# sczhou/CodeFormer

Hardware: AMD Instinct MI355X
Metric: aligned 512x512 faces/sec (whole node) at w=0.5 (higher is better)
Workload: dtype f32; 1 GPU; BASELINE config 2 (IEEE fp32 arithmetic): 16 faces/GPU, w=0.5, adain, seed-0 random-init weights; global_batch=16, parallelism=single GPU, precision=fp32

## Files before the change

### codeformer_amd/csrc/cf_wf43.hip

```cpp
#include <cstdlib>
#include <cstring>
#include <type_traits>

#include "cf_conv_parts.h"




namespace {

constexpr int F4_TH = 16, F4_TW = 16;
constexpr int F4_PW = F4_TW + 2;
constexpr int F4_NPIX = (F4_TH + 2) * F4_PW;
constexpr int F4_SLOTS = F4_NPIX + 4;
constexpr int F4_DUMMY = F4_NPIX;
constexpr int F4_NT = 16;
constexpr int F4_PATCH_FLOATS = F4_SLOTS * CF_BK;
constexpr int F4_PS = F4_NT * CF_BK;
constexpr int F4_V_FLOATS = 36 * F4_PS;
constexpr int F4_M_FLOATS = 36 * 8 * 64;
constexpr int F4_TAB = 256;
constexpr int F4_TAB_32 = 512;
constexpr int F4_LDS_FLOATS = 2 * F4_PATCH_FLOATS + F4_V_FLOATS + 2 * F4_TAB;
static_assert(F4_M_FLOATS <= 2 * F4_PATCH_FLOATS + F4_V_FLOATS, "epilogue staging must fit the patch buffers + V");
static_assert(F4_LDS_FLOATS * 4 <= 81920, "LDS budget of two workgroups per CU");
constexpr int F4_LDS_FLOATS_16 = 2 * F4_M_FLOATS;
static_assert(F4_LDS_FLOATS_16 >= F4_LDS_FLOATS && F4_LDS_FLOATS_16 * 4 <= 163840, "LDS budget of the 16-wave form");
constexpr int F4_LDS_FLOATS_32 = 2 * F4_SLOTS * 32 + 36 * F4_NT * 32 + 2 * F4_TAB_32;
static_assert(F4_LDS_FLOATS_32 >= F4_LDS_FLOATS_16 && F4_LDS_FLOATS_32 * 4 <= 163840, "LDS budget of the 32-channel-slab form");

typedef _Float16 f4_f16x4 __attribute__((ext_vector_type(4)));
typedef float f4_f32x2 __attribute__((ext_vector_type(2)));
typedef unsigned f4_u32x4 __attribute__((ext_vector_type(4)));
typedef unsigned f4_u32x2 __attribute__((ext_vector_type(2)));

__device__ __forceinline__ __amdgpu_buffer_rsrc_t f4_rsrc(const void* p, unsigned bytes) {
  return __builtin_amdgcn_make_buffer_rsrc(const_cast<void*>(p), 0, bytes, 0x00020000);
}
__device__ __forceinline__ f32x4 f4_ld128(__amdgpu_buffer_rsrc_t r, unsigned voff, unsigned soff) {
  return __builtin_bit_cast(f32x4, __builtin_amdgcn_raw_buffer_load_b128(r, (int)voff, (int)soff, 0));
}
__device__ __forceinline__ f4_f32x2 f4_ld64(__amdgpu_buffer_rsrc_t r, unsigned voff, unsigned soff) {
  return __builtin_bit_cast(f4_f32x2, __builtin_amdgcn_raw_buffer_load_b64(r, (int)voff, (int)soff, 0));
}
__device__ __forceinline__ void f4_st64(f4_f32x2 v, __amdgpu_buffer_rsrc_t r, unsigned voff, unsigned soff) {
  __builtin_amdgcn_raw_buffer_store_b64(__builtin_bit_cast(f4_u32x2, v), r, (int)voff, (int)soff, 0);
}

struct F4Args {
  const float* in0;
  const float* in1;
  int c0, c1, cin, nchunks;
  int batch, h, w;
  int cout;
  int prologue, epilogue;
  const float* pro_scale;
  const float* pro_shift;
  const float* weight;
  const float* bias;
  const float* res;
  const float* sft_scale;
  float sft_w;
  float acc_scale;
  const float* sft_w_img;
  const float* act_scale;
  float* out;
  double* stats_out;
  int stats_cpg, nparts;
  int tiles_x, tiles_per_img, ntn;
  int nt_out;
};
static_assert(sizeof(F4Args) == 168, "the kernarg block is 168 bytes (160 before sft_w_img, which found no padding to take): its size feeds the register allocation of every instantiation, so a change is re-checked with tools/kernel_resources.py");

__device__ __forceinline__ int f4_vs(int ty) { return (0x78 >> (2 * ty)) & 3; }

__device__ __forceinline__ unsigned f4_vu(unsigned lq, unsigned p, unsigned t) { return (lq & 1u) + 2u * (((t >> 1) + 4u * (lq >> 1) + p) & 7u); }

template <int PRO, int EPI, int NW, int KS, bool F32, int UPF = 0>
__global__ __launch_bounds__(NW * 64, 4) void wf43_kernel(const F4Args a) {
  constexpr bool UP = UPF == 2;
  constexpr bool GUP = UPF == 1;
  static_assert(UPF == 0 || (F32 && NW == 16 && KS == 32 && PRO == CF_PRO_NONE && EPI == CF_EPI_NONE), "the upsampling forms: fp32 operands on 32-channel slabs, no prologue, no epilogue operand");
  constexpr int NPW = UP ? 13 : 18;
  constexpr int NXI = UP ? 5 : 6;
  constexpr int OS = UP ? 2 : 1;
  static_assert(KS == 16 || (KS == 32 && NW == 16), "32-channel slabs need the LDS of the 16-wave form");
  constexpr int F4_THREADS = NW * 64;
  constexpr int F4_BN = NW * 8;
  constexpr int TWV = KS / 4;
  constexpr int QPP = KS / 4;
  constexpr int GT = F4_THREADS - TWV * 64;
  constexpr int F4_APT = 384 * QPP / GT;
  constexpr int PSTEP = GT / QPP;
  constexpr int SLOTB = KS * 4;
  constexpr int PATCHF = F4_SLOTS * KS;
  constexpr int PSK = F4_NT * KS;
  extern __shared__ __attribute__((aligned(16))) float smem[];
  float* const V = smem + 2 * PATCHF;
  constexpr int VBUF = 36 * PSK;
  constexpr int TABN = KS == 32 ? F4_TAB_32 : F4_TAB;
  float* const tab = V + VBUF;

  const int tid = threadIdx.x;
  const int lane = tid & 63;
  const int wave = __builtin_amdgcn_readfirstlane(tid >> 6);

  const int bid = cf_xcd_tile(blockIdx.x, gridDim.x);
  const int ntile = bid % a.ntn;
  const int mt = bid / a.ntn;
  const int n0 = ntile * F4_BN;
  const int b = mt / a.tiles_per_img;
  const int rt = mt - b * a.tiles_per_img;
  const int blocks = a.tiles_per_img >> 2;
  const int phase = UP ? rt / blocks : 0;
  const int pa = phase >> 1, pb = phase & 1;
  const int blk = UP ? rt - phase * blocks : rt;
  const int tyw = blk / a.tiles_x;
  const int y0 = tyw * F4_TH;
  const int x0 = (blk - tyw * a.tiles_x) * F4_TW;
  const int n = a.cin / KS;

  constexpr bool affine = PRO == CF_PRO_AFFINE || PRO == CF_PRO_AFFINE_SWISH;
  if (affine) {
    for (int i = tid; i < a.cin; i += F4_THREADS) {
      tab[i] = a.pro_scale[(size_t)b * a.cin + i];
      tab[TABN + i] = a.pro_shift[(size_t)b * a.cin + i];
    }
  }
  float act_s, act_is, act_s02;
  cf_act_scales<!affine>(a.act_scale, b, act_s, act_is, act_s02);

  const int py0 = y0 - 1 + pa, px0 = x0 - 1 + pb;
  const int pix_origin = py0 * a.w + px0;
  auto item = [&](unsigned u, int j, unsigned& rel, bool& valid) __attribute__((always_inline)) {
    const unsigned p = u + (unsigned)(PSTEP * j);
    const unsigned hy = (p * 3641u) >> 16;
    const unsigned hx = p - 18u * hy;
    const int iy = py0 + (int)hy, ix = px0 + (int)hx;
    valid = (int)(p < (unsigned)F4_NPIX) & (int)((unsigned)iy < (unsigned)a.h) & (int)((unsigned)ix < (unsigned)a.w);
    if constexpr (GUP) {
      const unsigned sy = valid ? (unsigned)iy : (unsigned)(y0 + 8), sx = valid ? (unsigned)ix : (unsigned)(x0 + 8);
      rel = (sy >> 1) * ((unsigned)a.w >> 1) + (sx >> 1);
    } else {
      rel = valid ? hy * (unsigned)a.w + hx : (unsigned)(9 * a.w + 9);
    }
  };
  const size_t img0 = (size_t)b * a.h * a.w;
  const unsigned img_px = (unsigned)(a.h * a.w);
  const size_t img0_in = GUP ? img0 / 4 : img0;
  const unsigned img_px_in = GUP ? img_px / 4 : img_px;
  const __amdgpu_buffer_rsrc_t rs_in0 = f4_rsrc(a.in0 + img0_in * a.c0, img_px_in * (unsigned)a.c0 * 4u);
  const __amdgpu_buffer_rsrc_t rs_in1 = f4_rsrc(a.c1 ? a.in1 + img0_in * a.c1 : a.in0, img_px_in * (unsigned)a.c1 * 4u);
  constexpr bool HALVES = F4_APT >= 6;
  constexpr int RAN = HALVES ? F4_APT / 2 : F4_APT;
  f32x4 ra[RAN], rb[HALVES ? RAN : 1];
  auto load_A_range = [&](int chunk, auto j0c, auto j1c) __attribute__((always_inline)) {
    constexpr int J0 = decltype(j0c)::value, J1 = decltype(j1c)::value;
    const int c = chunk * KS;
    const bool first = c < a.c0;
    const unsigned cs = (unsigned)(first ? a.c0 : a.c1);
    const unsigned soff = (unsigned)(first ? c : c - a.c0) * 4u;
    unsigned tl = (unsigned)tid - (unsigned)(TWV * 64);
    asm volatile("" : "+v"(tl));
    const unsigned k4x = (tl % (unsigned)QPP) * 4u;
#pragma unroll
    for (int j = J0; j < J1; ++j) {
      unsigned rel;
      bool valid;
      item(tl / (unsigned)QPP, j, rel, valid);
      const unsigned voff = (__umul24(GUP ? rel : (unsigned)(pix_origin + (int)rel), cs) + k4x) * 4u;
      (HALVES && j >= RAN ? rb[j % RAN] : ra[j % RAN]) = first ? f4_ld128(rs_in0, voff, soff) : f4_ld128(rs_in1, voff, soff);
    }
  };
  auto load_A = [&](int chunk) __attribute__((always_inline)) { load_A_range(chunk, std::integral_constant<int, 0>{}, std::integral_constant<int, F4_APT>{}); };
  auto store_patch_range = [&](int chunk, auto j0c, auto j1c) __attribute__((always_inline)) {
    constexpr int J0 = decltype(j0c)::value, J1 = decltype(j1c)::value;
    unsigned tl = (unsigned)tid - (unsigned)(TWV * 64);
    asm volatile("" : "+v"(tl));
    const unsigned k4 = tl % (unsigned)QPP, slot = tl / (unsigned)QPP;
    char* const pb = reinterpret_cast<char*>(smem + (chunk & 1) * PATCHF) + (((slot & ~3u) | ((slot ^ (slot >> 2)) & 3u)) * (unsigned)SLOTB + k4 * 16u);
    f32x4 sc = {1.f, 1.f, 1.f, 1.f}, sh = {0.f, 0.f, 0.f, 0.f};
    if (affine) {
      sc = *reinterpret_cast<const f32x4*>(tab + chunk * KS + k4 * 4);
      sh = *reinterpret_cast<const f32x4*>(tab + TABN + chunk * KS + k4 * 4);
    }
#pragma unroll
    for (int j = J0; j < J1; ++j) {
      unsigned rel;
      bool valid;
      item(slot, j, rel, valid);
      const f32x4 v = cf_pro_apply4<PRO, true>(HALVES && j >= RAN ? rb[j % RAN] : ra[j % RAN], sc, sh, act_s, act_s02, valid);
      if (j < F4_APT - 1 || slot + (unsigned)(PSTEP * j) < (unsigned)F4_NPIX) *reinterpret_cast<f32x4*>(pb + j * (PSTEP * SLOTB)) = v;
    }
  };

  auto store_patch = [&](int chunk) __attribute__((always_inline)) { store_patch_range(chunk, std::integral_constant<int, 0>{}, std::integral_constant<int, F4_APT>{}); };

  const int tg = (wave >> (KS == 32 ? 2 : 1)) & 1;
  float* t_hi;
  float* t_lo;
  auto row_pass = [&](const f4_f32x2 (&zz)[6], int pos) __attribute__((always_inline)) {
    f4_f32x2 v[6];
    v[0] = (zz[0] + zz[4]) * 0.25f - zz[2] * 1.0625f;
    const f4_f32x2 e1 = zz[4] * 0.25f - zz[2];
    const f4_f32x2 o1 = zz[3] * 0.125f - zz[1] * 0.5f;
    v[1] = e1 + o1;
    v[2] = e1 - o1;
    const f4_f32x2 e2 = zz[4] * 0.5f - zz[2] * 0.125f;
    const f4_f32x2 o2 = zz[3] - zz[1] * 0.25f;
    v[3] = e2 + o2;
    v[4] = e2 - o2;
    v[5] = (zz[1] + zz[5]) * 0.25f - zz[3] * 1.0625f;
#pragma unroll
    for (int nu = 0; nu < 6; ++nu) {
      if (F32) {
        t_hi[(pos + nu) * PSK] = v[nu][0];
        t_lo[(pos + nu) * PSK] = v[nu][1];
      } else {
        float hi, lo;
        cf_split_pair(v[nu][0], v[nu][1], hi, lo);
        t_hi[(pos + nu) * PSK] = hi;
        t_lo[(pos + nu) * PSK] = lo;
      }
    }
  };
  auto bt42 = [](auto xi, f4_f32x2 d0, f4_f32x2 d1, f4_f32x2 d2, f4_f32x2 d3, f4_f32x2 d4) __attribute__((always_inline)) {
    constexpr int XI = decltype(xi)::value;
    if constexpr (XI == 0) return (d0 + d3) - (d1 + d2) * 1.5f;
    else if constexpr (XI == 1) return (d1 + d3) - d2 * 2.5f;
    else if constexpr (XI == 2) return (d3 - d2) - d1 * 2.f;
    else if constexpr (XI == 3) return (d2 - d1) * 0.5f + d3;
    else return (d1 + d4) - (d2 + d3) * 1.5f;
  };
  auto row_pass42 = [&](const f4_f32x2 (&zz)[5], int pos) __attribute__((always_inline)) {
    f4_f32x2 v[5];
    v[0] = bt42(std::integral_constant<int, 0>{}, zz[0], zz[1], zz[2], zz[3], zz[4]);
    v[1] = bt42(std::integral_constant<int, 1>{}, zz[0], zz[1], zz[2], zz[3], zz[4]);
    v[2] = bt42(std::integral_constant<int, 2>{}, zz[0], zz[1], zz[2], zz[3], zz[4]);
    v[3] = bt42(std::integral_constant<int, 3>{}, zz[0], zz[1], zz[2], zz[3], zz[4]);
    v[4] = bt42(std::integral_constant<int, 4>{}, zz[0], zz[1], zz[2], zz[3], zz[4]);
#pragma unroll
    for (int nu = 0; nu < 5; ++nu) {
      t_hi[(pos + nu) * PSK] = v[nu][0];
      t_lo[(pos + nu) * PSK] = v[nu][1];
    }
  };
  auto transform = [&](int chunk, auto mid) __attribute__((always_inline)) {
    const char* const pb = reinterpret_cast<const char*>(smem + (chunk & 1) * PATCHF);
    unsigned ln = (unsigned)lane;
    asm volatile("" : "+v"(ln));
    constexpr int TG0 = UP ? 15 : 18;
    const unsigned t_tile = KS == 32 ? 4u * (unsigned)(wave & 3) + (ln >> 4) : 8u * (unsigned)(wave & 1) + (ln >> 3);
    const unsigned t_cp = KS == 32 ? ln & 15u : ln & 7u;
    const unsigned t_ty = t_tile >> 2, t_tx = t_tile & 3u;
    constexpr unsigned SH = KS == 32 ? 7 : 6;
    const unsigned t_base = (4u << SH) * (18u * t_ty + t_tx) + t_cp * 8u;
    const unsigned tb0 = 2u * t_ty + t_tx;
    unsigned tk[4];
#pragma unroll
    for (int k = 0; k < 4; ++k) tk[k] = t_base | (((tb0 + k) & 3u) << SH);
    if (F32) {
      const unsigned lq0 = (2u * t_cp) & 3u, j = t_cp >> 1;
      if (KS == 32) {
        t_hi = V + (tg * TG0) * PSK + t_tile * 32 + f4_vu(lq0, j >> 1, t_tile) * 2u + (j & 1u);
        t_lo = V + (tg * TG0) * PSK + t_tile * 32 + f4_vu(lq0 + 1u, j >> 1, t_tile) * 2u + (j & 1u);
      } else {
        t_hi = V + (tg * TG0) * PSK + t_tile * CF_BK + ((lq0 ^ (unsigned)f4_vs((int)t_ty)) << 2) + j;
        t_lo = V + (tg * TG0) * PSK + t_tile * CF_BK + (((lq0 + 1u) ^ (unsigned)f4_vs((int)t_ty)) << 2) + j;
      }
    } else if (KS == 32) {
      const unsigned lq = t_cp >> 2, e = t_cp & 3u;
      t_hi = V + (tg * TG0) * PSK + t_tile * 32 + f4_vu(lq, e >> 1, t_tile) * 2u + (e & 1u);
      t_lo = V + (tg * TG0) * PSK + t_tile * 32 + f4_vu(lq, 2u + (e >> 1), t_tile) * 2u + (e & 1u);
    } else {
      t_hi = V + (tg * TG0) * PSK + t_tile * CF_BK + (((t_cp >> 1) ^ (unsigned)f4_vs((int)t_ty)) << 2) + (t_cp & 1u);
      t_lo = t_hi + 2;
    }
    auto px = [&](int r, int j) __attribute__((always_inline)) {
      const int q = 2 * r + j;
      return *reinterpret_cast<const f4_f32x2*>(pb + (4 << SH) * (4 * r + (q >> 2)) + (tk[q >> 2] ^ (((unsigned)q & 3u) << SH)));
    };
    if constexpr (UP) {
      auto xi_pass = [&](auto xi) __attribute__((always_inline)) {
        constexpr int XI = decltype(xi)::value;
        f4_f32x2 z[5];
#pragma unroll
        for (int j = 0; j < 5; ++j) {
          const f4_f32x2 zero = {0.f, 0.f};
          z[j] = bt42(xi, XI == 0 ? px(0, j) : zero, px(1, j), px(2, j), px(3, j), XI == 4 ? px(4, j) : zero);
        }
        __builtin_amdgcn_sched_barrier(0);
        row_pass42(z, (XI >= 3 ? XI - 3 : XI) * 5);
        __builtin_amdgcn_sched_barrier(0);
      };
      if (tg == 0) {
        xi_pass(std::integral_constant<int, 0>{});
        xi_pass(std::integral_constant<int, 1>{});
        mid();
        __builtin_amdgcn_sched_barrier(0);
        xi_pass(std::integral_constant<int, 2>{});
      } else {
        xi_pass(std::integral_constant<int, 3>{});
        mid();
        __builtin_amdgcn_sched_barrier(0);
        xi_pass(std::integral_constant<int, 4>{});
      }
    } else if (tg == 0) {
      {
        f4_f32x2 z[6];
#pragma unroll
        for (int j = 0; j < 6; ++j) z[j] = (px(0, j) + px(4, j)) * 0.25f - px(2, j) * 1.0625f;
        __builtin_amdgcn_sched_barrier(0);
        row_pass(z, 0);
      }
      __builtin_amdgcn_sched_barrier(0);
      {
        f4_f32x2 zp[6], zm[6];
#pragma unroll
        for (int j = 0; j < 6; ++j) {
          const f4_f32x2 e = px(4, j) * 0.25f - px(2, j);
          const f4_f32x2 o = px(3, j) * 0.125f - px(1, j) * 0.5f;
          zp[j] = e + o;
          zm[j] = e - o;
          if (j == 2) __builtin_amdgcn_sched_barrier(0);
        }
        __builtin_amdgcn_sched_barrier(0);
        row_pass(zp, 6);
        __builtin_amdgcn_sched_barrier(0);
        mid();
        __builtin_amdgcn_sched_barrier(0);
        row_pass(zm, 12);
      }
    } else {
      {
        f4_f32x2 z[6];
#pragma unroll
        for (int j = 0; j < 6; ++j) z[j] = (px(1, j) + px(5, j)) * 0.25f - px(3, j) * 1.0625f;
        __builtin_amdgcn_sched_barrier(0);
        row_pass(z, 12);
      }
      __builtin_amdgcn_sched_barrier(0);
      {
        f4_f32x2 zp[6], zm[6];
#pragma unroll
        for (int j = 0; j < 6; ++j) {
          const f4_f32x2 e = px(4, j) * 0.5f - px(2, j) * 0.125f;
          const f4_f32x2 o = px(3, j) - px(1, j) * 0.25f;
          zp[j] = e + o;
          zm[j] = e - o;
          if (j == 2) __builtin_amdgcn_sched_barrier(0);
        }
        __builtin_amdgcn_sched_barrier(0);
        row_pass(zp, 0);
        __builtin_amdgcn_sched_barrier(0);
        mid();
        __builtin_amdgcn_sched_barrier(0);
        row_pass(zm, 6);
      }
    }
  };

  const int m_g = wave / (NW / 2), m_nb = wave % (NW / 2);
  f32x4 acc[NPW];
#pragma unroll
  for (int i = 0; i < NPW; ++i) acc[i] = f32x4{0.f, 0.f, 0.f, 0.f};
  const __amdgpu_buffer_rsrc_t rs_w = f4_rsrc(a.weight, (UP ? 100u : 36u) * (unsigned)a.cin * (unsigned)a.cout * 4u);
  const unsigned w_pos = (unsigned)a.cin * (unsigned)a.cout * 4u;
  const unsigned w_chunk = (unsigned)(a.cout * KS) * 4u;
  const unsigned w_s0 = (unsigned)(18 * m_g) * w_pos + (unsigned)(n0 / 16 + m_nb) * (unsigned)(64 * KS);
  constexpr std::integral_constant<int, 4> nb4{};
  unsigned lane16;
  f32x4 bq[4];
  auto load_B = [&](int chunk, int i, auto nb) __attribute__((always_inline)) {
    bq[i % decltype(nb)::value] = f4_ld128(rs_w, lane16, w_s0 + (unsigned)i * w_pos + (unsigned)chunk * w_chunk);
  };
  auto set_lane16 = [&]() __attribute__((always_inline)) {
    unsigned ln = (unsigned)lane;
    asm volatile("" : "+v"(ln));
    lane16 = ln * 16u;
  };
  const float* a_base;
  f32x4 va[4];
  auto mfma = [&](float a0, float a1, float b0, float b1, f32x4& c) __attribute__((always_inline)) {
    c = __builtin_amdgcn_mfma_f32_16x16x16f16(__builtin_bit_cast(f4_f16x4, f4_f32x2{a0, a1}), __builtin_bit_cast(f4_f16x4, f4_f32x2{b0, b1}), c, 0, 0, 0);
  };
  auto mma_stage = [&](int chunk, auto na, auto after_last_B) __attribute__((always_inline)) {
    constexpr int NA = decltype(na)::value;
    {
      unsigned ln = (unsigned)lane;
      asm volatile("" : "+v"(ln));
      const unsigned t15 = ln & 15u;
      a_base = V + (18 * m_g) * PSK + t15 * CF_BK + (((ln >> 4) ^ (unsigned)f4_vs((int)(t15 >> 2))) << 2);
      lane16 = ln * 16u;
    }
    auto read_A = [&](int i) __attribute__((always_inline)) { va[i % NA] = *reinterpret_cast<const f32x4*>(a_base + i * PSK); };
    read_A(0);
    read_A(1);
#pragma unroll
    for (int i = 0; i < 18; i += 2) {
      if (NA == 4 && i + 2 < 18) {
        read_A(i + 2);
        read_A(i + 3);
      }
      __builtin_amdgcn_sched_barrier(0);
      const f32x4 a0 = va[i % NA], a1 = va[(i + 1) % NA], b0 = bq[i % 4], b1 = bq[(i + 1) % 4];
      if (F32) {
#pragma unroll
        for (int j = 0; j < 4; ++j) {
          acc[i] = __builtin_amdgcn_mfma_f32_16x16x4f32(a0[j], b0[j], acc[i], 0, 0, 0);
          acc[i + 1] = __builtin_amdgcn_mfma_f32_16x16x4f32(a1[j], b1[j], acc[i + 1], 0, 0, 0);
        }
      } else {
        mfma(a0[2], a0[3], b0[0], b0[1], acc[i]);
        mfma(a1[2], a1[3], b1[0], b1[1], acc[i + 1]);
        mfma(a0[0], a0[1], b0[2], b0[3], acc[i]);
        mfma(a1[0], a1[1], b1[2], b1[3], acc[i + 1]);
        mfma(a0[0], a0[1], b0[0], b0[1], acc[i]);
        mfma(a1[0], a1[1], b1[0], b1[1], acc[i + 1]);
      }
      if (NA == 2 && i + 2 < 18) {
        read_A(i + 2);
        read_A(i + 3);
      }
      if (i + 4 < 18) {
        load_B(chunk, i + 4, nb4);
        load_B(chunk, i + 5, nb4);
      }
      if (i + 4 == 16) after_last_B();
      __builtin_amdgcn_sched_barrier(0);
    }
  };
  typedef _Float16 f4_f16x8 __attribute__((ext_vector_type(8)));
  f32x4 xb[3][2], xa[1][2];
  const int p_g = NPW * m_g;
  const int p_nb = m_nb;
  const bool p_last = !UP || m_g == 0;
  const unsigned w_s32 = (unsigned)(p_g + 25 * phase) * w_pos + (unsigned)(n0 / 16 + p_nb) * (unsigned)(64 * KS);
  auto load_B32 = [&](int chunk, int i) __attribute__((always_inline)) {
    const unsigned so = w_s32 + (unsigned)i * w_pos + (unsigned)chunk * w_chunk;
    xb[i % 3][0] = f4_ld128(rs_w, lane16, so);
    xb[i % 3][1] = f4_ld128(rs_w, lane16 + 16u, so);
  };
  auto mma_stage32 = [&](int chunk) __attribute__((always_inline)) {
    unsigned ao[4];
    {
      unsigned ln = (unsigned)lane;
      asm volatile("" : "+v"(ln));
      const unsigned t15 = ln & 15u, lq = ln >> 4;
#pragma unroll
      for (unsigned pp = 0; pp < 4; ++pp) ao[pp] = ((unsigned)p_g * (unsigned)PSK + t15 * 32u + f4_vu(lq, pp, t15) * 2u) * 4u;
      lane16 = ln * 32u;
    }
    const char* const vb = reinterpret_cast<const char*>(V);
    auto read_A = [&](int pos) __attribute__((always_inline)) {
      const f4_f32x2 p0 = *reinterpret_cast<const f4_f32x2*>(vb + ao[0] + pos * (PSK * 4)), p1 = *reinterpret_cast<const f4_f32x2*>(vb + ao[1] + pos * (PSK * 4));
      const f4_f32x2 p2 = *reinterpret_cast<const f4_f32x2*>(vb + ao[2] + pos * (PSK * 4)), p3 = *reinterpret_cast<const f4_f32x2*>(vb + ao[3] + pos * (PSK * 4));
      xa[0][0] = f32x4{p0[0], p0[1], p1[0], p1[1]};
      xa[0][1] = f32x4{p2[0], p2[1], p3[0], p3[1]};
    };
    auto mf = [&](f32x4 av, f32x4 bv, f32x4& c) __attribute__((always_inline)) {
      c = __builtin_amdgcn_mfma_f32_16x16x32_f16(__builtin_bit_cast(f4_f16x8, av), __builtin_bit_cast(f4_f16x8, bv), c, 0, 0, 0);
    };
    read_A(0);
#pragma unroll
    for (int i = 0; i < NPW; ++i) {
      __builtin_amdgcn_sched_barrier(0);
      if (F32) {
        if (i + 1 < NPW || p_last) {
#pragma unroll
          for (int j = 0; j < 8; ++j) {
            acc[i] = __builtin_amdgcn_mfma_f32_16x16x4f32(xa[0][j >> 2][j & 3], xb[i % 3][j >> 2][j & 3], acc[i], 0, 0, 0);
          }
        }
      } else {
        mf(xa[0][1], xb[i % 3][0], acc[i]);
        mf(xa[0][0], xb[i % 3][1], acc[i]);
        mf(xa[0][0], xb[i % 3][0], acc[i]);
      }
      if (i + 1 < NPW && (p_last || i + 1 < NPW - 1)) read_A(i + 1);
      if (i + 3 < NPW && (p_last || i + 3 < NPW - 1)) load_B32(chunk, i + 3);
      __builtin_amdgcn_sched_barrier(0);
    }
  };
  auto set_lane32 = [&]() __attribute__((always_inline)) {
    unsigned ln = (unsigned)lane;
    asm volatile("" : "+v"(ln));
    lane16 = ln * 32u;
  };
  constexpr std::integral_constant<int, 4> na4{};
  constexpr std::integral_constant<int, 4> na_gather{};
  auto feed = [&](int s) __attribute__((always_inline)) {
    if (s < n) {
      store_patch(s);
    }
  };

  if constexpr (KS == 32) {
    if (wave < TWV) {
      __syncthreads();
      __syncthreads();
      for (int s = 0; s < n; ++s) {
        transform(s, [&]() __attribute__((always_inline)) {
          set_lane32();
          load_B32(s, 0);
        });
        __builtin_amdgcn_sched_barrier(0);
        load_B32(s, 1);
        load_B32(s, 2);
        __builtin_amdgcn_sched_barrier(0);
        __syncthreads();
        mma_stage32(s);
        __builtin_amdgcn_sched_barrier(0);
        __syncthreads();
      }
    } else {
      constexpr std::integral_constant<int, 0> h0{};
      constexpr std::integral_constant<int, F4_APT / 2> h1{};
      constexpr std::integral_constant<int, F4_APT> h2{};
      auto feed2 = [&](int s) __attribute__((always_inline)) {
        if (s < n) {
          load_A_range(s, h1, h2);
          __builtin_amdgcn_sched_barrier(0);
          store_patch_range(s, h0, h1);
          __builtin_amdgcn_sched_barrier(0);
          store_patch_range(s, h1, h2);
        }
      };
      load_A_range(0, h0, h1);
      __syncthreads();
      feed2(0);
      if (n > 1) load_A_range(1, h0, h1);
      __syncthreads();
      for (int s = 0; s < n; ++s) {
        feed2(s + 1);
        __builtin_amdgcn_sched_barrier(0);
        set_lane32();
#pragma unroll
        for (int i = 0; i < 3; ++i) load_B32(s, i);
        __builtin_amdgcn_sched_barrier(0);
        __syncthreads();
        mma_stage32(s);
        __builtin_amdgcn_sched_barrier(0);
        if (s + 2 < n) load_A_range(s + 2, h0, h1);
        __builtin_amdgcn_sched_barrier(0);
        __syncthreads();
      }
    }
  } else if (wave < 4) {
    __syncthreads();
    __syncthreads();
    for (int s = 0; s < n; ++s) {
      transform(s, [&]() __attribute__((always_inline)) {
        set_lane16();
        load_B(s, 0, nb4);
        load_B(s, 1, nb4);
      });
      __builtin_amdgcn_sched_barrier(0);
      load_B(s, 2, nb4);
      load_B(s, 3, nb4);
      __builtin_amdgcn_sched_barrier(0);
      __syncthreads();
      mma_stage(s, na4, []() __attribute__((always_inline)) {});
      __builtin_amdgcn_sched_barrier(0);
      __syncthreads();
    }
  } else {
    constexpr std::integral_constant<int, 0> h0{};
    constexpr std::integral_constant<int, (HALVES ? F4_APT / 2 : F4_APT)> h1{};
    constexpr std::integral_constant<int, F4_APT> h2{};
    auto feedh = [&](int s) __attribute__((always_inline)) {
      if (s < n) {
        if (HALVES) load_A_range(s, h1, h2);
        __builtin_amdgcn_sched_barrier(0);
        store_patch_range(s, h0, h1);
        __builtin_amdgcn_sched_barrier(0);
        if (HALVES) store_patch_range(s, h1, h2);
      }
    };
    load_A_range(0, h0, h1);
    __syncthreads();
    feedh(0);
    if (n > 1) load_A_range(1, h0, h1);
    __syncthreads();
    int s = 0;
    for (; s + 2 < n; ++s) {
      feedh(s + 1);
      __builtin_amdgcn_sched_barrier(0);
      set_lane16();
#pragma unroll
      for (int i = 0; i < 4; ++i) load_B(s, i, nb4);
      __builtin_amdgcn_sched_barrier(0);
      __syncthreads();
      mma_stage(s, na_gather, [&]() __attribute__((always_inline)) { load_A_range(s + 2, h0, h1); });
      __builtin_amdgcn_sched_barrier(0);
      __syncthreads();
    }
    for (; s < n; ++s) {
      feedh(s + 1);
      __builtin_amdgcn_sched_barrier(0);
      set_lane16();
#pragma unroll
      for (int i = 0; i < 4; ++i) load_B(s, i, nb4);
      __builtin_amdgcn_sched_barrier(0);
      __syncthreads();
      mma_stage(s, na_gather, []() __attribute__((always_inline)) {});
      __builtin_amdgcn_sched_barrier(0);
      __syncthreads();
    }
  }

  float* const Mst = smem;
  const int e_cp = (lane & 31) + 32 * (wave >> 3), e_rh = lane >> 5, e_tp = wave & 7;
  const float acc_s = a.acc_scale * act_is;
  [[maybe_unused]] const float sft_w = EPI == CF_EPI_SFT ? cf_sft_weight(a.sft_w_img, a.sft_w, b) : 0.f;
  const int nn = n0 + 2 * e_cp;
  f4_f32x2 bias2 = {0.f, 0.f};
  if (a.bias) bias2 = *reinterpret_cast<const f4_f32x2*>(a.bias + nn);
  const unsigned e_rowc = (unsigned)(OS * OS * a.w) * (unsigned)a.cout * 4u;
  const unsigned e_px = (unsigned)(OS * a.cout) * 4u;
  const unsigned e_img = (unsigned)(OS * OS) * img_px * (unsigned)a.cout * 4u;
  const __amdgpu_buffer_rsrc_t rs_out = f4_rsrc(a.out + (size_t)(OS * OS) * img0 * a.cout, e_img);
  const __amdgpu_buffer_rsrc_t rs_res = f4_rsrc(EPI == CF_EPI_NONE ? a.out : a.res + img0 * a.cout, e_img);
  const __amdgpu_buffer_rsrc_t rs_sft = f4_rsrc(EPI == CF_EPI_SFT ? a.sft_scale + img0 * a.cout : a.out, e_img);
  const bool rh1 = e_rh != 0;
  const float ca1 = rh1 ? 0.25f : 1.f, ca2 = rh1 ? 4.f : 1.f, cb1 = rh1 ? 0.125f : 0.5f, cb2 = rh1 ? 8.f : 2.f;
  double psum = 0.0, psq = 0.0;
#pragma unroll
  for (int th = 0; th < 2; ++th) {
    unsigned e_zero = 0;
    asm volatile("" : "+v"(e_zero));
    const unsigned voff0 = (unsigned)(2 * e_rh) * e_rowc + (unsigned)(2 * e_cp) * 4u + e_zero;
    const unsigned soff0 = (unsigned)(y0 + 4 * (e_tp >> 1)) * e_rowc + (unsigned)(x0 + 4 * (2 * th + (e_tp & 1))) * e_px + (unsigned)n0 * 4u +
                           (UP ? (unsigned)(pa * 2 * a.w + pb) * (unsigned)a.cout * 4u : 0u);
    f4_f32x2 r0[2][4], r1[2][4];
#pragma unroll
    for (int aa = 0; aa < 2; ++aa)
#pragma unroll
      for (int c = 0; c < 4; ++c) {
        r0[aa][c] = r1[aa][c] = f4_f32x2{0.f, 0.f};
        if (EPI == CF_EPI_RESIDUAL || EPI == CF_EPI_SFT) r0[aa][c] = f4_ld64(rs_res, voff0, soff0 + aa * e_rowc + c * e_px);
      }
    __builtin_amdgcn_sched_barrier(0);
    if (th > 0) __syncthreads();
#pragma unroll
    for (int i = 0; i < NPW; ++i) {
      float* mp = Mst + ((NPW * m_g + i) * 8 + 2 * (lane >> 4)) * F4_BN + m_nb * 16 + (lane & 15);
      mp[0] = acc[i][2 * th];
      mp[F4_BN] = acc[i][2 * th + 1];
    }
    if (EPI == CF_EPI_SFT) {
#pragma unroll
      for (int aa = 0; aa < 2; ++aa)
#pragma unroll
        for (int c = 0; c < 4; ++c) r1[aa][c] = f4_ld64(rs_sft, voff0, soff0 + aa * e_rowc + c * e_px);
    }
    __syncthreads();
    const float* mq = Mst + e_tp * F4_BN + 2 * e_cp;
    auto col = [&](int nu, f4_f32x2& tA, f4_f32x2& tB) __attribute__((always_inline)) {
      auto m = [&](int xi) __attribute__((always_inline)) { return *reinterpret_cast<const f4_f32x2*>(mq + ((xi * NXI + nu) * 8) * F4_BN); };
      if constexpr (UP) {
        const f4_f32x2 m1 = m(1), m2 = m(2), m3 = m(3);
        const f4_f32x2 me = *reinterpret_cast<const f4_f32x2*>(mq + (((rh1 ? 4 : 0) * NXI + nu) * 8) * F4_BN);
        const f4_f32x2 x = m1 + m2 * ca1 + m3 * ca2, y = (m2 * cb1 + m3 * cb2) - m1;
        const f4_f32x2 xm = x + me, ym = y + me;
        tA = rh1 ? x : xm;
        tB = rh1 ? ym : y;
        return;
      }
      const f4_f32x2 m1 = m(1), m2 = m(2), m3 = m(3), m4 = m(4);
      const f4_f32x2 me = *reinterpret_cast<const f4_f32x2*>(mq + (((rh1 ? 5 : 0) * 6 + nu) * 8) * F4_BN);
      const f4_f32x2 s1 = m1 + m2, d1 = m1 - m2, s2 = m3 + m4, d2 = m3 - m4;
      const f4_f32x2 x = s1 * ca1 + s2 * ca2, y = d1 * cb1 + d2 * cb2;
      const f4_f32x2 xm = x + me, ym = y + me;
      tA = rh1 ? x : xm;
      tB = rh1 ? ym : y;
    };
    f4_f32x2 o[2][4];
    if constexpr (UP) {
      f4_f32x2 t[5][2];
#pragma unroll
      for (int nu = 0; nu < 5; ++nu) col(nu, t[nu][0], t[nu][1]);
#pragma unroll
      for (int aa = 0; aa < 2; ++aa) {
        o[aa][0] = (t[0][aa] + t[1][aa]) + (t[2][aa] + t[3][aa]);
        o[aa][1] = (t[2][aa] * 0.5f + t[3][aa] * 2.f) - t[1][aa];
        o[aa][2] = (t[2][aa] * 0.25f + t[3][aa] * 4.f) + t[1][aa];
        o[aa][3] = ((t[2][aa] * 0.125f + t[3][aa] * 8.f) - t[1][aa]) + t[4][aa];
      }
    } else {
      f4_f32x2 t0[2], ta[2], tb[2];
      col(0, t0[0], t0[1]);
      col(1, ta[0], ta[1]);
      col(2, tb[0], tb[1]);
#pragma unroll
      for (int aa = 0; aa < 2; ++aa) {
        const f4_f32x2 s = ta[aa] + tb[aa], d = ta[aa] - tb[aa];
        o[aa][0] = t0[aa] + s;
        o[aa][1] = d * 0.5f;
        o[aa][2] = s * 0.25f;
        o[aa][3] = d * 0.125f;
      }
      col(3, ta[0], ta[1]);
      col(4, tb[0], tb[1]);
      col(5, t0[0], t0[1]);
#pragma unroll
      for (int aa = 0; aa < 2; ++aa) {
        const f4_f32x2 s = ta[aa] + tb[aa], d = ta[aa] - tb[aa];
        o[aa][0] += s;
        o[aa][1] += d * 2.f;
        o[aa][2] += s * 4.f;
        o[aa][3] += d * 8.f + t0[aa];
      }
    }
    double dsum = 0.0, dsq = 0.0, dsum1 = 0.0, dsq1 = 0.0;
#pragma unroll
    for (int aa = 0; aa < 2; ++aa) {
      f4_f32x2 rs = {0.f, 0.f}, rq = {0.f, 0.f};
#pragma unroll
      for (int c = 0; c < 4; ++c) {
        f4_f32x2 v = o[aa][c] * acc_s + bias2;
        if (EPI == CF_EPI_RESIDUAL) v += r0[aa][c];
        else if (EPI == CF_EPI_SFT) v = r0[aa][c] + sft_w * (r0[aa][c] * r1[aa][c] + v);
        o[aa][c] = v;
        rs += v;
        rq += v * v;
      }
      dsum += (double)rs[0];
      dsq += (double)rq[0];
      dsum1 += (double)rs[1];
      dsq1 += (double)rq[1];
    }
    if (a.nt_out) {
#pragma unroll
      for (int aa = 0; aa < 2; ++aa)
#pragma unroll
        for (int c = 0; c < 4; ++c)
          __builtin_amdgcn_raw_buffer_store_b64(__builtin_bit_cast(f4_u32x2, o[aa][c]), rs_out, (int)voff0, (int)(soff0 + aa * e_rowc + c * e_px), 2);
    } else {
#pragma unroll
      for (int aa = 0; aa < 2; ++aa)
#pragma unroll
        for (int c = 0; c < 4; ++c) f4_st64(o[aa][c], rs_out, voff0, soff0 + aa * e_rowc + c * e_px);
    }
    if (a.stats_out) {
      const int cpg = a.stats_cpg;
      dsum += dsum1;
      dsq += dsq1;
      dsum += __shfl_xor(dsum, 32, 64);
      dsq += __shfl_xor(dsq, 32, 64);
      for (int o2 = 1; o2 * 2 < cpg; o2 <<= 1) {
        dsum += __shfl_xor(dsum, o2, 64);
        dsq += __shfl_xor(dsq, o2, 64);
      }
      psum = th == 0 ? dsum : psum + dsum;
      psq = th == 0 ? dsq : psq + dsq;
    }
  }
  if (a.stats_out) {
    const int cpg = a.stats_cpg;
    double* const sred = reinterpret_cast<double*>(smem);
    __syncthreads();
    if (e_rh == 0) {
      sred[(wave * 32 + (lane & 31)) * 2] = psum;
      sred[(wave * 32 + (lane & 31)) * 2 + 1] = psq;
    }
    __syncthreads();
    if (e_tp == 0 && e_rh == 0 && (nn % cpg) == 0) {
      double s0 = 0.0, s1 = 0.0;
#pragma unroll
      for (int wv = 0; wv < 8; ++wv) {
        s0 += sred[((wave + wv) * 32 + (lane & 31)) * 2];
        s1 += sred[((wave + wv) * 32 + (lane & 31)) * 2 + 1];
      }
      double* op = cf_gn_partial_ptr(a.stats_out, b, a.cout, cpg, nn, a.nparts, rt);
      op[0] = s0;
      op[1] = s1;
    }
  }
}

}

bool cf_wf43_k32(int cout, int cin) {
  static const bool enabled = [] {
    const char* w = getenv("CF_F43_WIDE");
    if (!w || !strcmp(w, "k32")) return true;
    if (!strcmp(w, "k16")) return false;
    fprintf(stderr, "libcodeformer_hip: CF_F43_WIDE=%s is not a form of the 16-wave F(4,3) workgroup (k32 | k16): using k32\n", w);
    return true;
  }();
  return cout % 128 == 0 && cin % 32 == 0 && enabled;
}

int cf_wf43_launch(const cf_conv_desc* d, hipStream_t stream, int* parts_query, const float* sft_w_img) {
  CF_REQUIRE(d->taps == 9 && d->stride == 1 && !d->in_nchw && !d->out_nchw &&
                 (d->bf16_mfma == CF_OPERAND_F16X2 || d->bf16_mfma == CF_OPERAND_F32),
             "cf_conv2d(winograd 2): F(4x4,3x3) covers 3x3 stride-1 NHWC convolutions with split-half or fp32 operands");
  const bool f32 = d->bf16_mfma == CF_OPERAND_F32;
  const bool sub = d->upsample == 2;
  CF_REQUIRE(!d->upsample || (f32 && d->prologue == CF_PRO_NONE && d->epilogue == CF_EPI_NONE && d->c1 == 0 && cf_wf43_k32(d->cout, d->c0)),
             "cf_conv2d(winograd 2, upsample): fp32 operands, one input with c0 %% 32 == 0, cout %% 128 == 0, no prologue / epilogue operand");
  CF_REQUIRE(!sub || (d->hin % F4_TH == 0 && d->win % F4_TW == 0 && d->hout == 2 * d->hin && d->wout == 2 * d->win),
             "cf_conv2d(winograd 2, upsample 2): needs an input of %dx%d multiples (got %dx%d)", F4_TH, F4_TW, d->hin, d->win);
  if (!f32)
    if (const int e = cf_require_acc_scale(d, "cf_conv2d(winograd 2)")) return e;
  CF_REQUIRE(!f32 || !d->act_scale, "cf_conv2d(winograd 2): fp32 operands take no activation range scale");
  CF_REQUIRE(d->hout % F4_TH == 0 && d->wout % F4_TW == 0, "cf_conv2d(winograd 2): needs an output of %dx%d multiples (got %dx%d)", F4_TH,
             F4_TW, d->hout, d->wout);
  CF_REQUIRE(d->cout % 64 == 0 && d->cout_pad == d->cout, "cf_conv2d(winograd 2): needs cout == cout_pad, a multiple of 64 (got %d / %d)",
             d->cout, d->cout_pad);
  CF_REQUIRE((long)d->hout * d->wout <= (1L << 21), "cf_conv2d(winograd 2): at most 2^21 pixels per image (got %dx%d)", d->hout, d->wout);
  CF_REQUIRE((long)d->hout * d->wout * (d->c0 > d->cout ? d->c0 : d->cout) * 4 < (1L << 31) && (long)d->hout * d->wout * d->c1 * 4 < (1L << 31),
             "cf_conv2d(winograd 2): an image of a tensor must stay below 2^31 bytes (%dx%d, %d / %d / %d channels)", d->hout, d->wout, d->c0, d->c1, d->cout);
  const int tab_max = cf_wf43_k32(d->cout, d->c0 + d->c1) ? F4_TAB_32 : F4_TAB;
  CF_REQUIRE(d->c0 + d->c1 <= tab_max, "cf_conv2d(winograd 2): at most %d input channels in this form (got %d)", tab_max, d->c0 + d->c1);
  CF_REQUIRE(cf_epi_is_quad_triple(d), "cf_conv2d(winograd 2): epilogues are none / residual / SFT");
  CF_REQUIRE(cf_dense_zero_pad(d) && d->split_k < 1, "cf_conv2d(winograd 2): reads / writes dense tensors with zero padding, no split_k");
  CF_REQUIRE(d->stats_cpg == 0 || (d->stats_cpg <= 64 && (d->stats_cpg & (d->stats_cpg - 1)) == 0 && d->stats_cpg >= 2),
             "cf_conv2d(winograd 2): stats_cpg %d (a power of two, 2..64)", d->stats_cpg);
  F4Args a;
  cf_fill_conv_args(a, d, sft_w_img);
  a.nchunks = a.cin / CF_BK;
  a.h = d->hout;
  a.w = d->wout;
  a.acc_scale = f32 ? 1.f : d->acc_scale;
  a.act_scale = d->act_scale;
  a.stats_cpg = d->stats_cpg > 0 ? d->stats_cpg : 2;
  a.tiles_x = d->wout / F4_TW;
  a.tiles_per_img = a.tiles_x * (d->hout / F4_TH);
  a.nparts = a.tiles_per_img;
  const bool wide = d->cout % 128 == 0;
  const bool k32 = cf_wf43_k32(d->cout, d->c0 + d->c1);
  CF_REQUIRE(!k32 || d->c0 % 32 == 0, "cf_conv2d(winograd 2): with cout %% 128 == 0 and cin %% 32 == 0 the concat boundary must be a multiple of 32 (c0 = %d)", d->c0);
  a.ntn = d->cout / (wide ? 128 : 64);
  a.nt_out = cf_nt_store((long)d->batch * d->hout * d->wout * d->cout * 4);
  if (sub) {
    a.h = d->hin;
    a.w = d->win;
    a.tiles_x = d->win / F4_TW;
  }
  if (parts_query) {
    *parts_query = a.nparts;
    return CF_OK;
  }
  const size_t lds = (k32 ? F4_LDS_FLOATS_32 : wide ? F4_LDS_FLOATS_16 : F4_LDS_FLOATS) * sizeof(float);
  const dim3 grid(a.tiles_per_img * d->batch * a.ntn), block(wide ? 1024 : 512);
  if (d->upsample) {
    CF_LDS_ATTR((wf43_kernel<CF_PRO_NONE, CF_EPI_NONE, 16, 32, true, 1>), F4_LDS_FLOATS_32 * sizeof(float));
    CF_LDS_ATTR((wf43_kernel<CF_PRO_NONE, CF_EPI_NONE, 16, 32, true, 2>), F4_LDS_FLOATS_32 * sizeof(float));
    if (sub) hipLaunchKernelGGL((wf43_kernel<CF_PRO_NONE, CF_EPI_NONE, 16, 32, true, 2>), grid, block, lds, stream, a);
    else hipLaunchKernelGGL((wf43_kernel<CF_PRO_NONE, CF_EPI_NONE, 16, 32, true, 1>), grid, block, lds, stream, a);
    CF_CHECK_LAUNCH("cf_conv2d(winograd F(4,3) / F(4,2) fp32, upsampling forms)");
    return CF_OK;
  }
  auto launch = [&](auto pro, auto epi, auto op) {
    constexpr int P = decltype(pro)::value, E = decltype(epi)::value;
    constexpr bool O = decltype(op)::value;
    CF_LDS_ATTR((wf43_kernel<P, E, 8, 16, O>), F4_LDS_FLOATS * sizeof(float));
    CF_LDS_ATTR((wf43_kernel<P, E, 16, 16, O>), F4_LDS_FLOATS_16 * sizeof(float));
    CF_LDS_ATTR((wf43_kernel<P, E, 16, 32, O>), F4_LDS_FLOATS_32 * sizeof(float));
    if (k32) hipLaunchKernelGGL((wf43_kernel<P, E, 16, 32, O>), grid, block, lds, stream, a);
    else if (wide) hipLaunchKernelGGL((wf43_kernel<P, E, 16, 16, O>), grid, block, lds, stream, a);
    else hipLaunchKernelGGL((wf43_kernel<P, E, 8, 16, O>), grid, block, lds, stream, a);
  };
  cf_with_prologue(d->prologue, [&](auto pro) {
    cf_with_epilogue(d->epilogue, [&](auto epi) {
      if (f32) launch(pro, epi, std::true_type{});
      else launch(pro, epi, std::false_type{});
    });
  });
  CF_CHECK_LAUNCH("cf_conv2d(winograd F(4,3) f16x2)");
  return CF_OK;
}
```

Baseline: 356.5 faces/s.

## Precompute packed halo-gather geometry per thread and split off the tail round

Instead of recomputing pixel coordinates, bounds checks and row offsets for every gathered halo item on every channel chunk, each loader thread now packs per-item row/column offsets and a validity bit into a few 10-bit fields once, then reuses them across chunks. The last partial round is separated into a tail item loaded only by waves that cover it, so full rounds drop the per-item range check. The feed order is also reshuffled to interleave the tail load with the first patch stores. This trades a few extra live registers for less integer address arithmetic in the gather loop, and adds risk around the clamped coordinates and the packed field widths.

```diff
diff --git a/codeformer_amd/csrc/cf_wf43.hip b/codeformer_amd/csrc/cf_wf43.hip
--- a/codeformer_amd/csrc/cf_wf43.hip
+++ b/codeformer_amd/csrc/cf_wf43.hip
@@ -13,7 +13,6 @@
 constexpr int F4_PW = F4_TW + 2;
 constexpr int F4_NPIX = (F4_TH + 2) * F4_PW;
 constexpr int F4_SLOTS = F4_NPIX + 4;
-constexpr int F4_DUMMY = F4_NPIX;
 constexpr int F4_NT = 16;
 constexpr int F4_PATCH_FLOATS = F4_SLOTS * CF_BK;
 constexpr int F4_PS = F4_NT * CF_BK;
@@ -90,7 +89,6 @@
   constexpr int TWV = KS / 4;
   constexpr int QPP = KS / 4;
   constexpr int GT = F4_THREADS - TWV * 64;
-  constexpr int F4_APT = 384 * QPP / GT;
   constexpr int PSTEP = GT / QPP;
   constexpr int SLOTB = KS * 4;
   constexpr int PATCHF = F4_SLOTS * KS;
@@ -131,13 +129,46 @@
   cf_act_scales<!affine>(a.act_scale, b, act_s, act_is, act_s02);
 
   const int py0 = y0 - 1 + pa, px0 = x0 - 1 + pb;
+  constexpr int F4_NFULL = F4_NPIX / PSTEP;
+  constexpr int F4_APT = F4_NFULL + 1;
+  static_assert(F4_NPIX % PSTEP != 0 && F4_APT * PSTEP >= F4_NPIX, "full rounds + one tail round cover the halo patch");
+  constexpr int PPW = 64 / QPP;
+  const bool tail_wave = (wave - TWV) * PPW + F4_NFULL * PSTEP < F4_NPIX;
+  auto grow = [](int j) constexpr { return GUP ? 0 : (PSTEP * j / F4_PW < 15 ? PSTEP * j / F4_PW : 15); };
+  static_assert((PSTEP - 1 + F4_PW - 1) / F4_PW + 1 <= 16, "an item's rows fit the four-bit row field");
+  const int geo_rs = GUP ? a.w >> 1 : a.w;
+  const int geo_org = GUP ? ((y0 >> 1) - 1) * (a.w >> 1) + (x0 >> 1) - 1 : py0 * a.w + px0;
+  constexpr int GW = (F4_APT + 2) / 3;
+  constexpr bool GEO = EPI != CF_EPI_SFT;
+  unsigned geo[GW];
+  auto field = [&](unsigned u, int j) __attribute__((always_inline)) {
+      const unsigned p = u + (unsigned)(PSTEP * j);
+      const unsigned hy = (p * 3641u) >> 16;
+      const unsigned hx = p - 18u * hy;
+      const int iy = py0 + (int)hy, ix = px0 + (int)hx;
+      const bool valid = (int)((unsigned)iy < (unsigned)a.h) & (int)((unsigned)ix < (unsigned)a.w);
+      const int cy = min(max(iy, 0), a.h - 1), cx = min(max(ix, 0), a.w - 1);
+      const unsigned fy = GUP ? (unsigned)((cy >> 1) - (y0 >> 1) + 1) : (unsigned)(cy - py0 - grow(j));
+      const unsigned fx = GUP ? (unsigned)((cx >> 1) - (x0 >> 1) + 1) : (unsigned)(cx - px0);
+      return fy | fx << 4 | (valid ? 0x200u : 0u);
+  };
+  auto build_geo = [&]() __attribute__((always_inline)) {
+    if constexpr (GEO) {
+      const unsigned u = ((unsigned)tid - (unsigned)(TWV * 64)) / (unsigned)QPP;
+#pragma unroll
+      for (int k = 0; k < GW; ++k) geo[k] = 0;
+#pragma unroll
+      for (int j = 0; j < F4_NFULL; ++j) geo[j / 3] |= field(u, j) << (10 * (j % 3));
+      if (tail_wave && u + (unsigned)(PSTEP * F4_NFULL) < (unsigned)F4_NPIX) geo[F4_NFULL / 3] |= field(u, F4_NFULL) << (10 * (F4_NFULL % 3));
+    }
+  };
   const int pix_origin = py0 * a.w + px0;
   auto item = [&](unsigned u, int j, unsigned& rel, bool& valid) __attribute__((always_inline)) {
     const unsigned p = u + (unsigned)(PSTEP * j);
     const unsigned hy = (p * 3641u) >> 16;
     const unsigned hx = p - 18u * hy;
     const int iy = py0 + (int)hy, ix = px0 + (int)hx;
-    valid = (int)(p < (unsigned)F4_NPIX) & (int)((unsigned)iy < (unsigned)a.h) & (int)((unsigned)ix < (unsigned)a.w);
+    valid = (int)((unsigned)iy < (unsigned)a.h) & (int)((unsigned)ix < (unsigned)a.w);
     if constexpr (GUP) {
       const unsigned sy = valid ? (unsigned)iy : (unsigned)(y0 + 8), sx = valid ? (unsigned)ix : (unsigned)(x0 + 8);
       rel = (sy >> 1) * ((unsigned)a.w >> 1) + (sx >> 1);
@@ -151,28 +182,46 @@
   const unsigned img_px_in = GUP ? img_px / 4 : img_px;
   const __amdgpu_buffer_rsrc_t rs_in0 = f4_rsrc(a.in0 + img0_in * a.c0, img_px_in * (unsigned)a.c0 * 4u);
   const __amdgpu_buffer_rsrc_t rs_in1 = f4_rsrc(a.c1 ? a.in1 + img0_in * a.c1 : a.in0, img_px_in * (unsigned)a.c1 * 4u);
-  constexpr bool HALVES = F4_APT >= 6;
-  constexpr int RAN = HALVES ? F4_APT / 2 : F4_APT;
-  f32x4 ra[RAN], rb[HALVES ? RAN : 1];
+  constexpr int RAN = F4_NFULL > 1 ? F4_NFULL / 2 : 1;
+  f32x4 ra[RAN], rb[F4_NFULL > RAN ? F4_NFULL - RAN : 1], rtl;
+  auto geo_opaque = [&]() __attribute__((always_inline)) {
+#pragma unroll
+    for (int k = 0; k < (GEO ? GW : 0); ++k) asm volatile("" : "+v"(geo[k]));
+  };
   auto load_A_range = [&](int chunk, auto j0c, auto j1c) __attribute__((always_inline)) {
     constexpr int J0 = decltype(j0c)::value, J1 = decltype(j1c)::value;
     const int c = chunk * KS;
     const bool first = c < a.c0;
-    const unsigned cs = (unsigned)(first ? a.c0 : a.c1);
+    const unsigned cs4 = (unsigned)(first ? a.c0 : a.c1) * 4u;
     const unsigned soff = (unsigned)(first ? c : c - a.c0) * 4u;
     unsigned tl = (unsigned)tid - (unsigned)(TWV * 64);
     asm volatile("" : "+v"(tl));
-    const unsigned k4x = (tl % (unsigned)QPP) * 4u;
-#pragma unroll
-    for (int j = J0; j < J1; ++j) {
-      unsigned rel;
-      bool valid;
-      item(tl / (unsigned)QPP, j, rel, valid);
-      const unsigned voff = (__umul24(GUP ? rel : (unsigned)(pix_origin + (int)rel), cs) + k4x) * 4u;
-      (HALVES && j >= RAN ? rb[j % RAN] : ra[j % RAN]) = first ? f4_ld128(rs_in0, voff, soff) : f4_ld128(rs_in1, voff, soff);
-    }
-  };
-  auto load_A = [&](int chunk) __attribute__((always_inline)) { load_A_range(chunk, std::integral_constant<int, 0>{}, std::integral_constant<int, F4_APT>{}); };
+    const unsigned k16 = (tl % (unsigned)QPP) * 16u;
+    geo_opaque();
+    auto load_item = [&](int j) __attribute__((always_inline)) {
+      if constexpr (!GEO) {
+        unsigned rel;
+        bool valid;
+        item(tl / (unsigned)QPP, j, rel, valid);
+        const unsigned voff = __umul24(GUP ? rel : (unsigned)(pix_origin + (int)rel), cs4) + k16;
+        (j == F4_NFULL ? rtl : j >= RAN ? rb[j - RAN] : ra[j]) = first ? f4_ld128(rs_in0, voff, soff) : f4_ld128(rs_in1, voff, soff);
+        return;
+      }
+      const unsigned g = geo[j / 3] >> (10 * (j % 3));
+      const unsigned org = (unsigned)(geo_org + grow(j) * geo_rs);
+      unsigned rel = __umul24(g & 15u, (unsigned)geo_rs) + ((g >> 4) & 31u);
+      asm("" : "+v"(rel));
+      const unsigned voff = __umul24(rel + org, cs4) + k16;
+      (j == F4_NFULL ? rtl : j >= RAN ? rb[j - RAN] : ra[j]) = first ? f4_ld128(rs_in0, voff, soff) : f4_ld128(rs_in1, voff, soff);
+    };
+#pragma unroll
+    for (int j = J0; j < (J1 < F4_NFULL ? J1 : F4_NFULL); ++j) load_item(j);
+    if constexpr (J1 == F4_APT) {
+      if (tail_wave) {
+        if (tl / (unsigned)QPP + (unsigned)(PSTEP * F4_NFULL) < (unsigned)F4_NPIX) load_item(F4_NFULL);
+      }
+    }
+  };
   auto store_patch_range = [&](int chunk, auto j0c, auto j1c) __attribute__((always_inline)) {
     constexpr int J0 = decltype(j0c)::value, J1 = decltype(j1c)::value;
     unsigned tl = (unsigned)tid - (unsigned)(TWV * 64);
@@ -184,17 +233,41 @@
       sc = *reinterpret_cast<const f32x4*>(tab + chunk * KS + k4 * 4);
       sh = *reinterpret_cast<const f32x4*>(tab + TABN + chunk * KS + k4 * 4);
     }
-#pragma unroll
-    for (int j = J0; j < J1; ++j) {
-      unsigned rel;
-      bool valid;
-      item(slot, j, rel, valid);
-      const f32x4 v = cf_pro_apply4<PRO, true>(HALVES && j >= RAN ? rb[j % RAN] : ra[j % RAN], sc, sh, act_s, act_s02, valid);
-      if (j < F4_APT - 1 || slot + (unsigned)(PSTEP * j) < (unsigned)F4_NPIX) *reinterpret_cast<f32x4*>(pb + j * (PSTEP * SLOTB)) = v;
-    }
-  };
-
-  auto store_patch = [&](int chunk) __attribute__((always_inline)) { store_patch_range(chunk, std::integral_constant<int, 0>{}, std::integral_constant<int, F4_APT>{}); };
+    geo_opaque();
+    auto store_item = [&](int j) __attribute__((always_inline)) {
+      bool valid = (geo[j / 3] >> (10 * (j % 3) + 9)) & 1u;
+      if constexpr (!GEO) {
+        unsigned rel;
+        item(slot, j, rel, valid);
+      }
+      *reinterpret_cast<f32x4*>(pb + j * (PSTEP * SLOTB)) =
+          cf_pro_apply4<PRO, !F32>(j == F4_NFULL ? rtl : j >= RAN ? rb[j - RAN] : ra[j], sc, sh, act_s, act_s02, valid);
+    };
+#pragma unroll
+    for (int j = J0; j < (J1 < F4_NFULL ? J1 : F4_NFULL); ++j) store_item(j);
+    if constexpr (J1 == F4_APT) {
+      if (tail_wave) {
+        if (slot + (unsigned)(PSTEP * F4_NFULL) < (unsigned)F4_NPIX) store_item(F4_NFULL);
+      }
+    }
+  };
+  auto feed = [&](int s) __attribute__((always_inline)) {
+    constexpr std::integral_constant<int, 0> h0{};
+    constexpr std::integral_constant<int, 1> h01{};
+    constexpr std::integral_constant<int, RAN> h1{};
+    constexpr std::integral_constant<int, F4_NFULL> hf{};
+    constexpr std::integral_constant<int, F4_APT> h2{};
+    if (s < n) {
+      load_A_range(s, h1, hf);
+      if constexpr (F4_NFULL == RAN) load_A_range(s, hf, h2);
+      __builtin_amdgcn_sched_barrier(0);
+      store_patch_range(s, h0, h01);
+      if constexpr (F4_NFULL > RAN) load_A_range(s, hf, h2);
+      store_patch_range(s, h01, h1);
+      __builtin_amdgcn_sched_barrier(0);
+      store_patch_range(s, h1, h2);
+    }
+  };
 
   const int tg = (wave >> (KS == 32 ? 2 : 1)) & 1;
   float* t_hi;
@@ -489,11 +562,6 @@
   };
   constexpr std::integral_constant<int, 4> na4{};
   constexpr std::integral_constant<int, 4> na_gather{};
-  auto feed = [&](int s) __attribute__((always_inline)) {
-    if (s < n) {
-      store_patch(s);
-    }
-  };
 
   if constexpr (KS == 32) {
     if (wave < TWV) {
@@ -515,24 +583,15 @@
       }
     } else {
       constexpr std::integral_constant<int, 0> h0{};
-      constexpr std::integral_constant<int, F4_APT / 2> h1{};
-      constexpr std::integral_constant<int, F4_APT> h2{};
-      auto feed2 = [&](int s) __attribute__((always_inline)) {
-        if (s < n) {
-          load_A_range(s, h1, h2);
-          __builtin_amdgcn_sched_barrier(0);
-          store_patch_range(s, h0, h1);
-          __builtin_amdgcn_sched_barrier(0);
-          store_patch_range(s, h1, h2);
-        }
-      };
+      constexpr std::integral_constant<int, RAN> h1{};
+      build_geo();
       load_A_range(0, h0, h1);
       __syncthreads();
-      feed2(0);
+      feed(0);
       if (n > 1) load_A_range(1, h0, h1);
       __syncthreads();
       for (int s = 0; s < n; ++s) {
-        feed2(s + 1);
+        feed(s + 1);
         __builtin_amdgcn_sched_barrier(0);
         set_lane32();
 #pragma unroll
@@ -566,25 +625,16 @@
     }
   } else {
     constexpr std::integral_constant<int, 0> h0{};
-    constexpr std::integral_constant<int, (HALVES ? F4_APT / 2 : F4_APT)> h1{};
-    constexpr std::integral_constant<int, F4_APT> h2{};
-    auto feedh = [&](int s) __attribute__((always_inline)) {
-      if (s < n) {
-        if (HALVES) load_A_range(s, h1, h2);
-        __builtin_amdgcn_sched_barrier(0);
-        store_patch_range(s, h0, h1);
-        __builtin_amdgcn_sched_barrier(0);
-        if (HALVES) store_patch_range(s, h1, h2);
-      }
-    };
+    constexpr std::integral_constant<int, RAN> h1{};
+    build_geo();
     load_A_range(0, h0, h1);
     __syncthreads();
-    feedh(0);
+    feed(0);
     if (n > 1) load_A_range(1, h0, h1);
     __syncthreads();
     int s = 0;
     for (; s + 2 < n; ++s) {
-      feedh(s + 1);
+      feed(s + 1);
       __builtin_amdgcn_sched_barrier(0);
       set_lane16();
 #pragma unroll
@@ -596,7 +646,7 @@
       __syncthreads();
     }
     for (; s < n; ++s) {
-      feedh(s + 1);
+      feed(s + 1);
       __builtin_amdgcn_sched_barrier(0);
       set_lane16();
 #pragma unroll
```

After: 359.1 faces/s (median of 6 runs). No clear change (+0.7%).
